# G1OJS/PyFT8

Measured on AMD Instinct MI355X. Metric: FT8 15-s frames decoded/sec, higher is better.
Workload: dtype f32

## Files before the change

pyft8_amd/csrc/ft8rx.hip:

```cpp
#include <hip/hip_runtime.h>
#include <math.h>
#include <stdarg.h>
#include <stdio.h>
#include <stdlib.h>
#include <string.h>
#include <algorithm>
#include <map>
#include <new>
#include <string>
#include <type_traits>
#include <utility>
#include <vector>
#include "../../include/ft8rx.h"
#include "ft8_dev.h"

#define WL_MULT(i) ((i) == WL_BP0 ? 5 : (i) == WL_OSDNAN ? 10 : 1)
#define NF0MAX (FT8RX_MAX_F0 > 1024 ? 2048 : 1024)

#include "kernels/common.hpp"
#include "kernels/spectrogram.hpp"
#include "kernels/sync_search.hpp"
#include "kernels/llr.hpp"
#include "kernels/ap_patterns.hpp"
#include "kernels/bp.hpp"
#include "kernels/cycle_spectrum.hpp"
#include "kernels/fine_sync.hpp"
#include "kernels/osd.hpp"
#include "kernels/ap_calls.hpp"
#include "kernels/recall.hpp"
#include "kernels/report.hpp"
#include "kernels/ddc.hpp"
#include "kernels/ddc_wide.hpp"
#include "kernels/ddc_rat.hpp"
#include "kernels/blanker.hpp"
#include "kernels/synth.hpp"
#include "kernels/subtract.hpp"
#include "kernels/probes.hpp"
#include "host_messages.hpp"
#include "batch_plan.hpp"
#include "ddc_ring.hpp"
#include "ddc_wide_ring.hpp"
#include "ddc_rat_ring.hpp"
#include "optins.hpp"
#include "ilp_launch.hpp"

#define EV_EAGER_BYTES ((size_t)1 << 20)
#define HIPCHK(h, x) do { hipError_t _e = (x); if (_e != hipSuccess) { set_err(h, "%s failed: %s (%s:%d)", #x, hipGetErrorString(_e), __FILE__, __LINE__); return -2; } } while (0)

static std::vector<uint32_t> osd_trial_table(int S, int D, int T) {
    std::vector<uint32_t> t;
    const uint32_t N = OSD_NONE;
// ... 184 lines not shown
    if (e != hipSuccess) { set_err(h, "hipHostMalloc(%zu bytes) failed: %s", n * sizeof(T), hipGetErrorString(e)); return -2; }
    h->pinned.push_back(q); *p = (T*)q; if (dev) *dev = (T*)d; return 0;
}

enum WsGroup { WS_STAGING, WS_STAGING2, WS_MASK, WS_RECALL, WS_REPORTS, WS_PACKED, WS_SUB, WS_SUBD, WS_ONES, WS_DDC, WS_BLANK };
struct FirstUse {
    ft8rx_handle* h; WsGroup g; size_t nd, nh; int rc = 0;
    std::vector<void**> members;
    FirstUse(ft8rx_handle* h_, WsGroup g_) : h(h_), g(g_), nd(h_->allocs.size()), nh(h_->pinned.size()) {}
    template <typename T> void dev(T** p, size_t n) { if (!rc && !(rc = dalloc(h, p, n))) members.push_back((void**)p); }
    template <typename T> void host(T** p, size_t n, T** d = nullptr) {
        if (rc || (rc = halloc(h, p, n, d))) return;
        members.push_back((void**)p); if (d) members.push_back((void**)d);
    }
    int done() {
        if (!rc) { h->ready |= 1u << g; return 0; }
        while (h->allocs.size() > nd) { hipFree(h->allocs.back()); h->allocs.pop_back(); }
        while (h->pinned.size() > nh) { hipHostFree(h->pinned.back()); h->pinned.pop_back(); }
        for (void** m : members) *m = nullptr;
        return -2;
    }
};
static bool ws_ready(const ft8rx_handle* h, WsGroup g) { return (h->ready >> g) & 1u; }
#define FIRST_HIP(F, x) do { if (!(F).rc) { hipError_t _e = (x); if (_e != hipSuccess) { set_err((F).h, "%s failed: %s (%s:%d)", #x, hipGetErrorString(_e), __FILE__, __LINE__); (F).rc = -2; } } } while (0)

static int need_staging(ft8rx_handle* h, bool second = false) {
    const WsGroup g = second ? WS_STAGING2 : WS_STAGING;
    if (ws_ready(h, g)) return 0;
    FirstUse F(h, g);
    F.dev(second ? &h->d_audio2 : &h->d_audio, (size_t)h->max_frames * FT8RX_NSAMP);
    return F.done();
}

static void host_twiddle(int n, int count, std::vector<cpx>& w) {
    w.resize(count);
    for (int t = 0; t < count; t++) {
        double ang = (2.0 * M_PI * (double)t) / (double)n;
        w[t] = make_float2((float)cos(ang), (float)(-sin(ang)));
    }
}
template <typename T> static int upload(ft8rx_handle* h, const T** dst, const std::vector<T>& v) {
    T* p; if (dalloc(h, &p, v.size())) return -2;
    if (hipMemcpy(p, v.data(), v.size() * sizeof(T), hipMemcpyHostToDevice) != hipSuccess) { set_err(h, "table upload failed"); return -2; }
    *dst = p; return 0;
}

struct Scratch {
    ft8rx_handle* h;
    ~Scratch() { for (auto& c : h->arena) c.used = 0; }
    void* raw(size_t bytes) {
        bytes = (bytes + 255) & ~(size_t)255;
        if (!bytes) bytes = 256;
        for (auto& c : h->arena) if (c.cap - c.used >= bytes) { void* q = (char*)c.p + c.used; c.used += bytes; return q; }
        size_t largest = 0;
        for (auto& c : h->arena) if (c.cap > largest) largest = c.cap;
        size_t cap = bytes > 2 * largest ? bytes : 2 * largest;
        if (cap < ((size_t)1 << 20)) cap = (size_t)1 << 20;
        for (size_t i = 0; i < h->arena.size();) {
            if (h->arena[i].used == 0) { hipFree(h->arena[i].p); h->arena.erase(h->arena.begin() + i); } else i++;
        }
        void* q = nullptr;
        if (hipMalloc(&q, cap) != hipSuccess) { if (cap == bytes || hipMalloc(&q, bytes) != hipSuccess) return nullptr; cap = bytes; }
        h->arena.push_back({q, cap, bytes});
        return q;
    }
    template <typename T> T* get(size_t n) { return (T*)raw(n * sizeof(T)); }
// ... 125 lines not shown
    for (int i = 0; i < WL_N; i++) rc |= dalloc(h, &h->d_work[i], B * S * WL_MULT(i));
    rc |= dalloc(h, &h->d_wcount, (size_t)batchplan::MAX_CHUNKS * WL_N);
    rc |= dalloc(h, &h->d_apc, batchplan::MAX_CHUNKS);
    rc |= dalloc(h, &h->d_apcount, (size_t)batchplan::MAX_CHUNKS * 2);
    rc |= dalloc(h, &h->d_ev, B * FT8RX_EVENT_CAP);
    rc |= dalloc(h, &h->d_evcount, B);
    ResultSlot* const sl = h->slots;
    sl[0].rec = h->d_rec; sl[0].ncand = h->d_ncand; sl[0].ev = h->d_ev; sl[0].evcount = h->d_evcount;
    rc |= dalloc(h, &sl[1].rec, B * S);
    rc |= dalloc(h, &sl[1].ncand, B);
    rc |= dalloc(h, &sl[1].ev, B * FT8RX_EVENT_CAP);
    rc |= dalloc(h, &sl[1].evcount, B);
    const bool ev_compact = B * FT8RX_EVENT_CAP * sizeof(ft8rx_event) > EV_EAGER_BYTES;
    for (int k = 0; k < 2 && ev_compact; k++) rc |= dalloc(h, &sl[k].d_evoffs, B + 1);
    for (int k = 0; k < 2 && !rc; k++) {
        rc = halloc(h, &sl[k].h_rec, B * cfg->max_cands);
        if (!rc) rc = halloc(h, &sl[k].h_cnt, B);
        if (!rc) rc = halloc(h, &sl[k].h_ev, B * FT8RX_EVENT_CAP);
        if (!rc) rc = halloc(h, &sl[k].h_evc, B);
        if (!rc && ev_compact) rc = halloc(h, &sl[k].h_evpacked, B * FT8RX_EVENT_CAP, &sl[k].d_evpacked);
    }
    if (rc) { g_create_err = h->err; ft8rx_destroy(h); return -2; }
    std::vector<float> win(3840);
    for (int i = 0; i < 3840; i++) win[i] = (float)(0.5 + 0.5 * cos(M_PI * (double)(2 * i + 1 - 3840) / 3839.0));
    std::vector<double> taper(100);
    { double step = (0.0 - M_PI) / 99.0; for (int i = 0; i < 100; i++) { double y = (i == 99) ? 0.0 : (double)i * step + M_PI; taper[i] = 0.5 * (1.0 + cos(y)); } }
    std::vector<cpx> w;
    rc |= upload(h, &h->T.win, win);
    rc |= upload(h, &h->T.taper, taper);
    host_twiddle(1920, 1920, w);   rc |= upload(h, &h->T.W1920, w);
    host_twiddle(3840, FT8RX_GRID_COLS, w);    rc |= upload(h, &h->T.WR3840, w);
    host_twiddle(3200, 3200, w);   rc |= upload(h, &h->T.W3200, w);
    host_twiddle(96000, 96000, w); rc |= upload(h, &h->T.W96000, w);
    host_twiddle(300, 300, w);     rc |= upload(h, &h->T.W300, w);
    host_twiddle(320, 320, w);     rc |= upload(h, &h->T.W320, w);
    host_twiddle(192000, FT8RX_SPEC_BINS, w); rc |= upload(h, &h->T.WR192k, w);
    host_twiddle(32, 32, w);       rc |= upload(h, &h->T.W32, w);
    {
        std::vector<float> k32(1800);
        std::vector<cpx> cs(156), g1000(1000);
        for (int m = -900; m < 900; m++) {
            const int r = ((m % 100) + 100) % 100;
            k32[m + 900] = (r == 0) ? (m == 0 ? 32.0f : 0.0f) : (float)(sin(M_PI * (double)r / 100.0) / sin(M_PI * (double)m / 3200.0));
        }
        for (int sidx = 1; sidx < 7; sidx++) for (int q = 0; q <= 25; q++) {
            const double a = 2.0 * M_PI * (double)((q * sidx) % 100) / 100.0;
            cpx v = make_float2((float)cos(a), (float)sin(a));
            if (q == 0) v = make_float2(1.0f, 0.0f);
            cs[(sidx - 1) * 26 + q] = v;
        }
        for (int k = -150; k < 850; k++) {
            const int r = ((k % 100) + 100) % 100, j = (k - r) / 100;
            const double a = M_PI * (31.0 * (double)r - 100.0 * (double)j) / 3200.0;
            g1000[k + 150] = make_float2((float)cos(a), (float)sin(a));
        }
        std::vector<cpx> tw100(100);
        for (int m = 0; m < 100; m++) { const double a = -2.0 * M_PI * (double)m / 100.0; tw100[m] = make_float2((float)cos(a), (float)sin(a)); }
        rc |= upload(h, &h->T.K32, k32); rc |= upload(h, &h->T.CS100, cs); rc |= upload(h, &h->T.G1000, g1000); rc |= upload(h, &h->T.TW100, tw100);
    }
    if (rc) { g_create_err = h->err; ft8rx_destroy(h); return -2; }
    bool ok = true;
    ok &= hipMemcpyToSymbol(HIP_SYMBOL(d_CHK_N), FT8_CHK_N, sizeof(FT8_CHK_N)) == hipSuccess;
    ok &= hipMemcpyToSymbol(HIP_SYMBOL(d_CHK_V), FT8_CHK_V, sizeof(FT8_CHK_V)) == hipSuccess;
    {
        static uint8_t ev[522], ec[522]; static uint16_t ve[174][3];
        auto slot = [](int e) { const int c = FT8_EDGE_C[e], j = e - FT8_CHK_E0[c]; return j < 6 ? 83 * j + c : 498 + (c - 59); };
        for (int e = 0; e < 522; e++) { ev[slot(e)] = FT8_EDGE_V[e]; ec[slot(e)] = FT8_EDGE_C[e]; }
        for (int v = 0; v < 174; v++) for (int k = 0; k < 3; k++) ve[v][k] = (uint16_t)slot(FT8_VAR_E[v][k]);
        ok &= hipMemcpyToSymbol(HIP_SYMBOL(d_EDGE_V), ev, sizeof(ev)) == hipSuccess;
// ... 151 lines not shown
    const ResultSlot& sl = h->slots[slot];
    const bool weak = h->weak;
    const ft8rx_config cw = weak ? weak_config(h) : h->cfg;
    const ft8rx_config& c = weak ? cw : h->cfg;
    const size_t F = (size_t)f0;
    const int sh = cand_shift(c); const size_t S = (size_t)1 << sh, FS = F * S;
    const int16_t* audio = d_audio + F * FT8RX_NSAMP;
    float* grid = h->d_grid + F * FT8RX_GRID_ROWS * FT8RX_GRID_COLS;
    float* bs = h->d_best_score + F * NF0MAX; int32_t* bh = h->d_best_h0 + F * NF0MAX;
    ft8rx_record* rec = sl.rec + FS; int32_t* ncand = sl.ncand + F;
    float* llr0 = h->d_llr0 + FS * 174; float* saved = h->d_saved + FS * 5 * 174;
    Att* att0 = h->d_att0 + FS * 5; Att* attG = h->d_attG + FS * 2; Att* attB = h->d_attB + FS * 5; Att* attO = h->d_attO + FS * 10;
    cpx* A = reinterpret_cast<cpx*>(grid); cpx* spec = A + (size_t)B * 96000;
    ft8rx_event* ev = sl.ev + F * FT8RX_EVENT_CAP; int32_t* evc = sl.evcount + F;
#define STAGE(name) do { if (prof) { hipEventRecord(h->pev[h->pnames.size()], s); h->pnames.push_back(name); } } while (0)
    int32_t* wc = h->d_wcount + WL_N * chunk;
    WorkList wl[WL_N];
    for (int i = 0; i < WL_N; i++) { wl[i].items = h->d_work[i] + FS * WL_MULT(i); wl[i].count = wc + i; }
    STAGE("spectrogram");
    ft8rx_ilp_spectrogram(B, s, audio, grid, h->T);
    STAGE("sync");
    launch_sync(grid, bs, bh, c, B, s, weak);
    STAGE("topk");
    k_topk<<<B, 1024, 0, s>>>(bs, bh, rec, ncand, c, evc, wc, h->use_mask ? h->d_colmask + F * NF0MAX : nullptr);
    STAGE("grid_llr");
    const unsigned mt = (unsigned)h->msg_types;
    launch_mt(k_grid_llr, k_grid_llr_ext, mt, XCD_GRID(B, c.max_cands), s, grid, rec, ncand, llr0, c, nullptr, nullptr, nullptr, att0, ev, evc, B);
    k_worklist_att<<<(B * S * 5 + 255) / 256, 256, 0, s>>>(rec, ncand, att0, B, sh, wl[WL_BP0]);
    STAGE("bp_grid");
    launch_mt(k_bp, k_bp_ext, mt, ladder_grid(h, B * c.max_cands * 5), s, 0, llr0, rec, ncand, nullptr, att0, nullptr, ev, evc, c, c.bp_nc0_a, c.bp_iters_a, wl[WL_BP0], 0, 5);
    STAGE("select0");
    k_select0<<<(B * S + 255) / 256, 256, 0, s>>>(rec, ncand, att0, B, sh, wl[WL_FINE]);
    STAGE("cycle_fft");
    k_cyc_a<<<dim3(40, B), 256, 0, s>>>(audio, A, h->T);
    k_cyc_bc<<<dim3(CYC_BC_GRID, B), 256, 0, s>>>(A, spec, h->T);
    STAGE("fine");
    launch_fine(h, c, weak, ladder_grid(h, B * c.max_cands), s, spec, rec, ncand, llr0, nullptr, nullptr, nullptr, nullptr, wl[WL_FINE],
                c.h0_lo < FT8RX_MIN_H0_FD || c.h0_hi > FT8RX_MAX_H0_FD + 1);
    k_worklist<<<(B * S + 255) / 256, 256, 0, s>>>(rec, ncand, B, sh, wl[WL_BP1]);
    STAGE("bp_fine");
    const auto bp_fine = [&](int n_variants, const WorkList& work, int v0) {
        launch_mt(k_bp, k_bp_ext, mt, B * c.max_cands * n_variants, s, 1, llr0, rec, ncand, attG, attB, saved, ev, evc, c, c.bp_nc0_b, c.bp_iters_b,
                  work, v0, n_variants);
    };
    if (h->ladder_mode == 0) {
        bp_fine(1, wl[WL_BP1], 0);
        k_select1<<<(B * S + 255) / 256, 256, 0, s>>>(0, rec, ncand, attG, attB, B, c, wl[WL_BP1B]);
        bp_fine(1, wl[WL_BP1B], 1);
        k_select1<<<(B * S + 255) / 256, 256, 0, s>>>(1, rec, ncand, attG, attB, B, c, wl[WL_BP1C]);
        bp_fine(3, wl[WL_BP1C], 2);
        STAGE("select1");
        k_select1<<<(B * S + 255) / 256, 256, 0, s>>>(2, rec, ncand, attG, attB, B, c, wl[WL_OSD]);
    } else {
        bp_fine(5, wl[WL_BP1], 0);
        STAGE("select1");
        k_select1<<<(B * S + 255) / 256, 256, 0, s>>>(3, rec, ncand, attG, attB, B, c, wl[WL_OSD]);
    }
    STAGE("osd");
    launch_osd(h, mt, ladder_grid(h, B * c.max_cands * 10), s, 0, llr0, saved, attB, rec, ncand, attO, ev, evc, h->d_trials, h->n_trials,
               osd_nflip(c.osd_single, c.osd_triple), c.osd_max_hd, sh, wl[WL_OSD], wl[WL_OSDNAN]);
    STAGE("select2");
    k_select2<<<(B * S + 255) / 256, 256, 0, s>>>(rec, ncand, attO, B, sh);
    if (h->ap.np) {
        STAGE("ap_calls");
        ApCalls* apc = h->d_apc + chunk;
        if (h->ap_chunk_version[chunk] != h->ap_version) {
            k_ap_stage<<<1, 64, 0, s>>>(apc, h->ap);
            h->ap_chunk_version[chunk] = h->ap_version;
// ... 1507 lines not shown
    return sync_scores(h, grid, B, f0_lo, f0_hi, score, h0_idx, true);
}

static std::vector<int32_t> pack_triples(int n, const int32_t* frame, const int32_t* f0_idx, const int32_t* h0_idx) {
    std::vector<int32_t> trip(3 * (size_t)n);
    for (int i = 0; i < n; i++) { trip[3 * i] = frame[i]; trip[3 * i + 1] = f0_idx[i]; trip[3 * i + 2] = h0_idx[i]; }
    return trip;
}

int ft8rx_llr_grid(ft8rx_handle* h, const float* grid, int B, int n, const int32_t* frame, const int32_t* f0_idx,
                   const int32_t* h0_idx, float* llr, float* sd, int32_t* snr) {
    if (!h || !grid || B < 1 || B > h->max_frames || n < 1) return -1;
    ENTER(h);
    HIPCHK(h, hipMemcpy(h->d_grid, grid, sizeof(float) * (size_t)B * FT8RX_GRID_ROWS * FT8RX_GRID_COLS, hipMemcpyHostToDevice));
    const std::vector<int32_t> trip = pack_triples(n, frame, f0_idx, h0_idx);
    Scratch S{h};
    int32_t* d_trip = S.put(trip.data(), trip.size()); NEED(d_trip);
    float* d_llr = S.get<float>((size_t)n * 174); NEED(d_llr);
    float* d_sd = S.get<float>(n); NEED(d_sd);
    int32_t* d_snr = S.get<int32_t>(n); NEED(d_snr);
    k_grid_llr<<<n, 64, 0, h->stream>>>(h->d_grid, nullptr, nullptr, d_llr, h->cfg, d_trip, d_sd, d_snr, nullptr, nullptr, nullptr, n);
    HIPCHK(h, hipStreamSynchronize(h->stream));
    HIPCHK(h, hipMemcpy(llr, d_llr, sizeof(float) * (size_t)n * 174, hipMemcpyDeviceToHost));
    HIPCHK(h, hipMemcpy(sd, d_sd, sizeof(float) * n, hipMemcpyDeviceToHost));
    HIPCHK(h, hipMemcpy(snr, d_snr, sizeof(int32_t) * n, hipMemcpyDeviceToHost));
    return 0;
}

int ft8rx_cycle_spectrum(ft8rx_handle* h, const int16_t* audio, int B, float* spec) {
    if (!h || !audio || !spec || B < 1 || B > h->max_frames) return -1;
    ENTER(h);
    if (need_staging(h)) return -2;
    HIPCHK(h, hipMemcpy(h->d_audio, audio, sizeof(int16_t) * (size_t)B * FT8RX_NSAMP, hipMemcpyHostToDevice));
    k_cyc_a<<<dim3(40, B), 256, 0, h->stream>>>(h->d_audio, h->d_A, h->T);
    k_cyc_bc<<<dim3(CYC_BC_GRID, B), 256, 0, h->stream>>>(h->d_A, h->d_spec, h->T);
    HIPCHK(h, hipStreamSynchronize(h->stream));
    HIPCHK(h, hipMemcpy(spec, h->d_spec, sizeof(cpx) * (size_t)B * FT8RX_SPEC_BINS, hipMemcpyDeviceToHost));
    return 0;
}

static int fine_probe(ft8rx_handle* h, const float* spec, int B, int n, const int32_t* frame, const int32_t* f0_idx, const int32_t* h0_idx,
                      int32_t* ret, int32_t* ttweak, int32_t* ftweak, int32_t* nsync, float* llr, float* sd, int32_t* snr, float* sgrid, bool weak) {
    if (!h || !spec || B < 1 || B > h->max_frames || n < 1) return -1;
    if (weak) for (int i = 0; i < n; i++)
        if (frame[i] < 0 || frame[i] >= B || f0_idx[i] < 4 || f0_idx[i] >= FT8RX_MAX_F0 || h0_idx[i] < FT8RX_MIN_H0 || h0_idx[i] >= FT8RX_MAX_H0) {
            set_err(h, "ft8rx_fine_weak: triple %d (frame %d, f0 %d, h0 %d) outside [0, %d) x [4, %d) x [%d, %d)", i,
                    frame[i], f0_idx[i], h0_idx[i], B, FT8RX_MAX_F0, FT8RX_MIN_H0, FT8RX_MAX_H0); return -1; }
    ENTER(h);
    HIPCHK(h, hipMemcpy(h->d_spec, spec, sizeof(cpx) * (size_t)B * FT8RX_SPEC_BINS, hipMemcpyHostToDevice));
    const std::vector<int32_t> trip = pack_triples(n, frame, f0_idx, h0_idx);
    Scratch S{h};
    int32_t* d_trip = S.put(trip.data(), trip.size()); NEED(d_trip);
    float* d_llr = S.get<float>((size_t)n * 174); NEED(d_llr);
    HIPCHK(h, hipMemset(d_llr, 0, sizeof(float) * (size_t)n * 174));
    float* d_sd = S.get<float>(n); NEED(d_sd);
    int32_t* d_out = S.get<int32_t>((size_t)n * 5); NEED(d_out);
    float* d_sg = sgrid ? S.get<float>((size_t)n * 632) : nullptr; if (sgrid) NEED(d_sg);
    launch_fine(h, weak ? weak_config(h) : h->cfg, weak, n, h->stream, h->d_spec, nullptr, nullptr, d_llr, d_trip, d_out, d_sd, d_sg,
                WorkList{nullptr, nullptr}, true);
    HIPCHK(h, hipStreamSynchronize(h->stream));
    std::vector<int32_t> o((size_t)n * 5);
    HIPCHK(h, hipMemcpy(o.data(), d_out, sizeof(int32_t) * o.size(), hipMemcpyDeviceToHost));
    for (int i = 0; i < n; i++) { ret[i] = o[5 * i]; ttweak[i] = o[5 * i + 1]; ftweak[i] = o[5 * i + 2]; nsync[i] = o[5 * i + 3]; snr[i] = o[5 * i + 4]; }
    HIPCHK(h, hipMemcpy(llr, d_llr, sizeof(float) * (size_t)n * 174, hipMemcpyDeviceToHost));
    HIPCHK(h, hipMemcpy(sd, d_sd, sizeof(float) * n, hipMemcpyDeviceToHost));
    if (sgrid) HIPCHK(h, hipMemcpy(sgrid, d_sg, sizeof(float) * (size_t)n * 632, hipMemcpyDeviceToHost));
    return 0;
}
// ... 313 lines not shown
    ENTER(h);
    HIPCHK(h, hipStreamSynchronize(h->stream));
    if (subtract_workspaces(h, 0)) return -2;
    if (h->sig_cap < max_sigs) {
        ft8rx_subsig* p = nullptr;
        if (dalloc(h, &p, (size_t)h->max_frames * max_sigs)) return -2;
        h->d_sigs = p; h->sig_cap = max_sigs;
    }
    int nmax = 0;
    for (int f = 0; f < B; f++) {
        if (counts[f] < 0 || counts[f] > max_sigs) { set_err(h, "ft8rx_subtract: counts[%d] = %d outside [0, %d]", f, counts[f], max_sigs); return -1; }
        if (counts[f] > nmax) nmax = counts[f];
    }
    HIPCHK(h, hipMemcpyAsync(h->d_sigs, sigs, sizeof(ft8rx_subsig) * (size_t)B * max_sigs, hipMemcpyHostToDevice, h->stream));
    HIPCHK(h, hipMemcpyAsync(h->d_sigcnt, counts, sizeof(int32_t) * B, hipMemcpyHostToDevice, h->stream));
    const size_t n = (size_t)B * FT8RX_NSAMP;
    k_sub_to_f32<<<(unsigned)((n + 255) / 256), 256, 0, h->stream>>>(d_audio, h->d_wf, n);
    if (subtract_workspaces(h, refine)) return -2;
    const SubTables T{h->d_pulse, h->d_pc};
    Tables Tones = h->T;
    if (refine == 3) Tones.taper = h->d_ones;
    for (int s = 0; s < nmax; s++) {
        const SubSel sel{h->d_sigs, h->d_sigcnt, max_sigs, s};
        if (refine == 2) {
            k_subd_mix<<<dim3(SUBD_NZ / 256, B), 256, 0, h->stream>>>(h->d_wf, sel, h->d_zdec, h->d_subctx);
            sub_refine(h, B, sel, T, true);
            k_subd_model<<<dim3((SUBD_N + 255) / 256, B), 256, 0, h->stream>>>(sel, T, h->d_subctx, h->d_model);
            k_subd_accum<<<B, 256, 0, h->stream>>>(h->d_zdec, h->d_model, sel, h->d_subctx, h->d_adec);
            k_subd_apply<<<dim3(SUB_GRIDX, B), 256, 0, h->stream>>>(h->d_wf, sel, T, h->d_adec);
            continue;
        }
        if (refine == 1) sub_refine(h, B, sel, T, false);
        if (refine == 3) {
            k_cyc_a_f32<<<dim3(40, B), 256, 0, h->stream>>>(h->d_wf, h->d_A, h->T);
            k_cyc_bc<<<dim3(CYC_BC_GRID, B), 256, 0, h->stream>>>(h->d_A, h->d_spec, h->T);
            k_refine3<<<B, FINE_NT, 0, h->stream>>>(h->d_spec, sel, Tones);
        }
        sub_apply_fullrate(h, B, sel, T);
    }
    k_sub_to_i16<<<(unsigned)((n + 255) / 256), 256, 0, h->stream>>>(h->d_wf, d_audio, n);
    HIPCHK(h, hipGetLastError());
    if (audio_f32_out) HIPCHK(h, hipMemcpyAsync(audio_f32_out, h->d_wf, sizeof(float) * n, hipMemcpyDeviceToHost, h->stream));
    if (refine) HIPCHK(h, hipMemcpyAsync(sigs, h->d_sigs, sizeof(ft8rx_subsig) * (size_t)B * max_sigs, hipMemcpyDeviceToHost, h->stream));
    HIPCHK(h, hipStreamSynchronize(h->stream));
    return 0;
}

int ft8rx_encode_tones(const uint64_t* msg_lo, const uint64_t* msg_hi, int n, uint8_t* tones) {
    if (!msg_lo || !msg_hi || !tones || n < 0) return -1;
    for (int i = 0; i < n; i++) hostmsg::encode_tones(msg_lo[i], msg_hi[i], tones + (size_t)i * 79);
    return 0;
}

void* ft8rx_alloc_host(ft8rx_handle* h, uint64_t bytes) {
    if (!h || bytes == 0) return nullptr;
    void* p = nullptr;
    if (hipSetDevice(h->device) != hipSuccess || hipHostMalloc(&p, (size_t)bytes, hipHostMallocDefault) != hipSuccess) {
        set_err(h, "ft8rx_alloc_host: hipHostMalloc(%llu) failed", (unsigned long long)bytes);
        return nullptr;
    }
    return p;
}

int ft8rx_free_host(ft8rx_handle* h, void* p) {
    if (!p) return -1;
    const hipError_t e = hipHostFree(p);
    if (e != hipSuccess) { if (h) set_err(h, "hipHostFree failed: %s", hipGetErrorString(e)); return -2; }
    return 0;
// ... 138 lines not shown
```

pyft8_amd/csrc/kernels/common.hpp:

```cpp
#ifndef FT8RX_COMMON_HPP
#define FT8RX_COMMON_HPP

struct Tables {
    const float* win;
    const cpx* W1920;
    const cpx* WR3840;
    const cpx* W3200;
    const cpx* W96000;
    const cpx* W300;
    const cpx* W320;
    const cpx* WR192k;
    const cpx* W32;
    const double* taper;
    const float* K32;
    const cpx* CS100;
    const cpx* TW100;
    const cpx* G1000;
};

__device__ __constant__ int d_COSTAS[7] = {3, 1, 4, 0, 6, 5, 2};
__device__ __constant__ uint8_t d_PAYSYM[58] = {7,8,9,10,11,12,13,14,15,16,17,18,19,20,21,22,23,24,25,26,27,28,29,30,31,32,33,34,35,
    43,44,45,46,47,48,49,50,51,52,53,54,55,56,57,58,59,60,61,62,63,64,65,66,67,68,69,70,71};
struct WorkList { int32_t* items; int32_t* count; };

constexpr __host__ __device__ int cand_shift(int max_cands) { return max_cands <= 256 ? 8 : max_cands <= 512 ? 9 : max_cands <= 1024 ? 10 : 11; }
constexpr __host__ __device__ int cand_shift(const ft8rx_config& c) { return cand_shift(c.max_cands); }
FT8_DEV bool cand_live(int c, int B, int sh, const int32_t* ncand) { return c < (B << sh) && (c & ((1 << sh) - 1)) < ncand[c >> sh]; }

FT8_DEV bool xcd_frame_map(int L, int per, int B, int& frame, int& idx) {
    const int x = L & 7, j = L >> 3;
    frame = 8 * (j / per) + x; idx = j % per;
    return frame < B;
}
#define XCD_GRID(B, per) ((((B) + 7) / 8) * 8 * (per))
enum { WL_BP0 = 0, WL_FINE = 1, WL_BP1 = 2, WL_BP1B = 3, WL_BP1C = 4, WL_OSD = 5, WL_OSDNAN = 6, WL_N = 7 };

#define W6 ((double)(-0.16666667163372040f))

#ifndef FT8RX_ILP_UNIT
__device__ __constant__ int8_t d_AP_CQ[29]   = {0,0,0,0,0, 0,0,0,0,0, 0,0,0,0,0, 0,0,0,0,0, 0,0,0,0,0, 0,1,0,0};
__device__ __constant__ int8_t d_AP_END[3][19] = {{0,1, 1,1,1,1,1, 0,0,1,1,1, 0,1,0,1,0, 0,1},
                                                  {0,1, 1,1,1,1,1, 0,1,0,0,1, 0,1,0,0,0, 0,1},
                                                  {0,1, 1,1,1,1,1, 0,1,0,0,1, 0,0,1,0,0, 0,1}};
__device__ uint8_t  d_CHK_N[83];
__device__ int16_t  d_CHK_V[83][7];
// ... 195 lines not shown
```

pyft8_amd/csrc/kernels/cycle_spectrum.hpp:

```cpp
#ifndef FT8RX_CYCLE_SPECTRUM_HPP
#define FT8RX_CYCLE_SPECTRUM_HPP

FT8_DEV uint32_t cyc_a_pair(const int16_t* __restrict__ a, int at, int inb) { return *reinterpret_cast<const uint32_t*>(a + at) & (uint32_t)inb; }
FT8_DEV float2 cyc_a_pair(const float* __restrict__ a, int at, int inb) {
    const float2 v = *reinterpret_cast<const float2*>(a + at);
    return make_float2(__uint_as_float(__float_as_uint(v.x) & (uint32_t)inb), __uint_as_float(__float_as_uint(v.y) & (uint32_t)inb));
}
FT8_DEV cpx cyc_a_point(uint32_t raw) { return make_float2((float)(int16_t)(raw & 0xFFFFu), (float)(int16_t)(raw >> 16)); }
FT8_DEV cpx cyc_a_point(float2 raw) { return raw; }
template <class In, class Raw> FT8_DEV void cyc_a_load(const In* __restrict__ a, int n2b, int tid, Raw (&raw)[10]) {
#pragma unroll
    for (int q = 0; q < 10; q++) {
        const int i = tid + 256 * q, ic = i < 2400 ? i : 0;
        const int c = ic & 7, n1 = ic >> 3;
        const int m = 320 * n1 + n2b + c;
        const int inb = (2 * m < FT8RX_NSAMP) ? -1 : 0;
        raw[q] = cyc_a_pair(a, (2 * m) & inb, inb);
    }
}
template <class Raw> FT8_DEV void cyc_a_frame(const Raw (&raw)[10], cpx* bufA, cpx* bufB, cpx* __restrict__ out, const Tables& T, int n2b, int tid) {
#pragma unroll
    for (int q = 0; q < 10; q++) {
        const int i = tid + 256 * q;
        if (i < 2400) bufA[(i & 7) * 300 + (i >> 3)] = cyc_a_point(raw[q]);
    }
    cpx w[10];
#pragma unroll
    for (int q = 0; q < 10; q++) { const int i = tid + 256 * q, ic = i < 2400 ? i : 0; w[q] = T.W96000[(n2b + (ic & 7)) * (ic >> 3)]; }
    __syncthreads();
    cpx* r = lds_fft<300, 5, 5, 4, 3>(bufA, bufB, T.W300, 8, tid, 256);
#pragma unroll
    for (int q = 0; q < 10; q++) {
        const int i = tid + 256 * q;
        if (i < 2400) { const int c = i & 7, k1 = i >> 3; out[k1 * 320 + n2b + c] = cmul(r[c * 300 + k1], w[q]); }
    }
}
__global__ __launch_bounds__(256) void k_cyc_a(const int16_t* __restrict__ audio, cpx* __restrict__ A, Tables T) {
    __shared__ cpx bufA[8 * 300];
    __shared__ cpx bufB[8 * 300];
    static_assert(320 / 8 == 8 * 5, "the tile map below assumes 40 column tiles = 8 XCDs x 5");
    const int tile = (blockIdx.x & 7) * 5 + (blockIdx.x >> 3);
    const int f = blockIdx.y, tid = threadIdx.x, n2b = 8 * tile;
    uint32_t raw[10];
    cyc_a_load(audio + (size_t)f * FT8RX_NSAMP, n2b, tid, raw);
    cyc_a_frame(raw, bufA, bufB, A + (size_t)f * 96000, T, n2b, tid);
}

#define CYC_BC_BLOCKS 39
#define CYC_BC_GRID 40
FT8_DEV int cyc_bc_row(int b, int r) {
    if (b == CYC_BC_BLOCKS - 1) return (r == 0) ? 0 : 150;
    const int k1a = 1 + 4 * b;
    return (r < 4) ? k1a + r : 300 - (k1a + (r - 4));
}
FT8_DEV void cyc_bc_load(const cpx* __restrict__ in, int b, int tid, cpx (&v)[10]) {
#pragma unroll
    for (int q = 0; q < 10; q++) {
        const int i = tid + 256 * q, r = i / 320, c = i - 320 * r;
        v[q] = in[(size_t)cyc_bc_row(b, r) * 320 + c];
    }
}
FT8_DEV void cyc_bc_frame(const cpx (&v)[10], cpx* bufA, cpx* bufB, cpx* __restrict__ out, const Tables& T, int b, int tid) {
#pragma unroll
    for (int q = 0; q < 10; q++) bufA[tid + 256 * q] = v[q];
    __syncthreads();
    cpx* z = lds_fft<320, 8, 8, 5>(bufA, bufB, T.W320, 8, tid, 256);
    const bool special = (b == CYC_BC_BLOCKS - 1);
    constexpr int NK2 = (FT8RX_SPEC_BINS + 299) / 300;
    static_assert(NK2 <= 320, "k2 range of the 320-point row transforms");
    for (int i = tid; i < 8 * NK2; i += 256) {
        const int half = i / (4 * NK2), j = i - half * (4 * NK2), rr = j & 3, k2 = j >> 2;
        const int r = 4 * half + rr;
        int pr, pk2;
        if (special) {
            if (r >= 2) continue;
            pr = r;
            pk2 = (r == 0) ? ((320 - k2) % 320) : 319 - k2;
        } else {
            pr = (r < 4) ? r + 4 : r - 4;
            pk2 = 319 - k2;
        }
        const int k = cyc_bc_row(b, r) + 300 * k2;
        if (k >= FT8RX_SPEC_BINS) continue;
        const cpx p = z[r * 320 + k2], q = z[pr * 320 + pk2];
        const float er = 0.5f * (p.x + q.x), ei = 0.5f * (p.y - q.y);
        const float orr = 0.5f * (p.y + q.y), oi = 0.5f * (q.x - p.x);
        const cpx w = T.WR192k[k];
        out[k] = make_float2(er + (w.x * orr - w.y * oi), ei + (w.x * oi + w.y * orr));
    }
}
__global__ __launch_bounds__(256) void k_cyc_bc(const cpx* __restrict__ A, cpx* __restrict__ spec, Tables T) {
    __shared__ cpx bufA[8 * 320];
    __shared__ cpx bufB[8 * 320];
    static_assert(CYC_BC_GRID == 8 * 5 && CYC_BC_BLOCKS <= CYC_BC_GRID, "tile map: 40 slots = 8 XCDs x 5");
    const int f = blockIdx.y, tid = threadIdx.x, b = (blockIdx.x & 7) * 5 + (blockIdx.x >> 3);
    if (b >= CYC_BC_BLOCKS) return;
    cpx v[10];
    cyc_bc_load(A + (size_t)f * 96000, b, tid, v);
    cyc_bc_frame(v, bufA, bufB, spec + (size_t)f * FT8RX_SPEC_BINS, T, b, tid);
}

#endif
```

pyft8_amd/csrc/kernels/subtract.hpp:

```cpp
#ifndef FT8RX_SUBTRACT_HPP
#define FT8RX_SUBTRACT_HPP

#define SUB_L (79 * 1920)
#define SUB_NCH 128
#define SUB_CH (SUB_L / SUB_NCH)

struct SubTables { const double* pulse; const double* pc; };

FT8_DEV void sub_signal(const ft8rx_subsig& S, const double* __restrict__ cum , const SubTables& T, int m, float* sr, float* si) {
    const int n = m + 1920;
    const double dphi_peak = 6.283185307179586 / 1920.0;
    int ih = n / 1920; if (ih > 78) ih = 78;
    const int il = ih - 2 > 0 ? ih - 2 : 0;
    double acc = cum[il] * T.pc[5759];
    for (int i = il; i <= ih; i++) {
        int j = n - 1920 * i; if (j > 5759) j = 5759;
        acc += (double)S.tones[i] * T.pc[j];
    }
    double phi = dphi_peak * acc + 6.283185307179586 * (S.fHz - 0.5) * (double)n / 12000.0;
    if (n < 3840) phi += dphi_peak * T.pulse[1920 + n] * (double)S.tones[0];
    if (n >= 79 * 1920) phi += dphi_peak * T.pulse[n - 79 * 1920] * (double)S.tones[78];
    const double rev = phi * (1.0 / 6.283185307179586);
    const float fr = (float)(rev - floor(rev));
    const float s = __builtin_amdgcn_sinf(fr), c = __builtin_amdgcn_cosf(fr);
// ... 324 lines not shown
        if (lane == 0) { pr[wave][k] = vr; pi_[wave][k] = vi; }
    }
    __syncthreads();
    if (tid < 20) {
        const double sc = ok ? (double)SUBD_D / 192000.0 : 0.0;
        Ar[tid] = (float)(((pr[0][tid] + pr[1][tid]) + (pr[2][tid] + pr[3][tid])) * sc);
        Ai[tid] = (float)(((pi_[0][tid] + pi_[1][tid]) + (pi_[2][tid] + pi_[3][tid])) * sc);
    }
    __syncthreads();
    for (int m = tid; m <= SUBD_N; m += 256) {
        const float rv = (float)(SUBD_D * m) * (1.0f / 192000.0f);
        float er, ei;
        sub_bins_synth(Ar, Ai, __builtin_amdgcn_cosf(rv), __builtin_amdgcn_sinf(rv), &er, &ei);
        adec[(size_t)frame * (SUBD_N + 1) + m] = make_float2(er, ei);
    }
}

__global__ __launch_bounds__(256) void k_subd_apply(float* __restrict__ wf, SubSel sel, SubTables T, const float2* __restrict__ adec) {
    __shared__ SubModel M;
    const int frame = blockIdx.y;
    int s0;
    if (!sub_begin(sel, frame, &M, &s0) || !sub_fits(s0)) return;
    float* x = wf + (size_t)frame * FT8RX_NSAMP + s0;
    const float2* a = adec + (size_t)frame * (SUBD_N + 1);
    sub_walk(M, T, [&](int m, float sr, float si) {
        int md = m >> 5; if (md > SUBD_N - 1) md = SUBD_N - 1;
        const float2 a0 = a[md], a1 = a[md + 1];
        float fq = (float)(m - SUBD_D * md) * (1.0f / 32.0f); if (fq > 1.0f) fq = 1.0f;
        const float er = a0.x + fq * (a1.x - a0.x), ei = a0.y + fq * (a1.y - a0.y);
        x[m] = x[m] - 2.0f * (er * sr - ei * si);
    });
}

__global__ __launch_bounds__(256) void k_cyc_a_f32(const float* __restrict__ audio, cpx* __restrict__ A, Tables T) {
    __shared__ cpx bufA[8 * 300];
    __shared__ cpx bufB[8 * 300];
    const int tile = (blockIdx.x & 7) * 5 + (blockIdx.x >> 3);
    const int f = blockIdx.y, tid = threadIdx.x, n2b = 8 * tile;
    float2 raw[10];
    cyc_a_load(audio + (size_t)f * FT8RX_NSAMP, n2b, tid, raw);
    cyc_a_frame(raw, bufA, bufB, A + (size_t)f * 96000, T, n2b, tid);
}

__global__ __launch_bounds__(FINE_NT) void k_refine3(const cpx* __restrict__ spec, SubSel sel, Tables T) {
    __shared__ cpx z[3200];
    __shared__ cpx slice[FINE_SLICE];
    __shared__ cpx w400[400];
    __shared__ cpx w32[32];
    __shared__ __attribute__((aligned(8))) double dsum[12 * 21 * 2];
    const int frame = blockIdx.x, tid = threadIdx.x;
    if (sel.s >= sel.counts[frame]) return;
    ft8rx_subsig& S = sel.sigs[(size_t)frame * sel.max_sigs + sel.s];
    const int fb0 = (int)(0.5 + S.fHz * 16.0);
    const int tb0 = (int)(0.5 + S.tsec * 200.0);
    if (fb0 - 182 < 0 || fb0 - 182 + FINE_SLICE > FT8RX_SPEC_BINS) return;
    const cpx* Sg = spec + (size_t)frame * FT8RX_SPEC_BINS + (fb0 - 182);
    for (int i = tid; i < FINE_SLICE; i += FINE_NT) slice[i] = Sg[i];
    for (int i = tid; i < 400; i += FINE_NT) w400[i] = T.W3200[8 * i];
    if (tid < 32) w32[tid] = T.W32[tid];
    __syncthreads();
    cpx wq[8];
    sym32_twiddles(w32, tid & 3, wq);
    FT_DECL
    fine_fft(slice, 182, z, w400, T, tid, 0, 3200 FT_PASS);
#pragma unroll 1
    for (int r = 0; r < (12 * 21 * 4 + FINE_NT - 1) / FINE_NT; r++) {
        const int task = tid + FINE_NT * r, qd = task >> 2, n2 = task & 3;
        const bool valid = qd < 12 * 21;
        const int ti = valid ? qd / 21 : 0, sy = valid ? qd - 21 * ti : 0;
        const int blk = sy / 7, a = sy - 7 * blk;
        float mag[8];
        fine_sym_quad<7>(z, tb0 - 6 + ti + 32 * (36 * blk + a), n2, wq, mag);
        if (valid && n2 == 0) { double on, off; fine_onoff(mag, a, on, off); dsum[(ti * 21 + sy) * 2] = on; dsum[(ti * 21 + sy) * 2 + 1] = off; }
    }
// ... 29 lines not shown
```

Baseline: 87230.

## Restructure cycle FFT kernels into 16-column register tiles with precomputed twiddle tables

```diff
diff --git a/pyft8_amd/csrc/cyc_index.hpp b/pyft8_amd/csrc/cyc_index.hpp
--- /dev/null
+++ b/pyft8_amd/csrc/cyc_index.hpp
@@ -0,0 +1,59 @@
+#pragma once
+#include <cstdint>
+
+#if defined(__HIPCC__)
+#define CYC_HD __host__ __device__ constexpr
+#else
+#define CYC_HD constexpr
+#endif
+
+namespace cycidx {
+
+constexpr int A_COLS = 16, A_TILES = 320 / A_COLS, A_BLOCK = 256, A_G1 = 12 * A_COLS, A_G2 = 25 * A_COLS, A_E = 12;
+constexpr int A_ROUNDS = (A_G2 + A_BLOCK - 1) / A_BLOCK;
+static_assert(A_TILES * A_COLS == 320 && A_G1 <= A_BLOCK && A_ROUNDS == 2, "20 tiles of 16 columns; one stage-1 group, two stage-2 groups per thread");
+CYC_HD int a_in_row(int g1, int jp, int j) { return g1 / A_COLS + 12 * jp + 60 * j; }
+struct APoint { int n2, k1; };
+CYC_HD APoint a_point(int tile, int g2, int e) {
+    return APoint{A_COLS * tile + g2 % A_COLS, g2 / A_COLS + 25 * (e % 4) + 100 * (e / 4)};
+}
+CYC_HD int a_pos(int tile, int g2, int e) { return (tile * A_E + e) * A_G2 + g2; }
+constexpr int A_TABLE = A_TILES * A_E * A_G2;
+
+constexpr int BC_BLOCKS = 20, BC_SLOTS = 16, BC_HALF = BC_SLOTS / 2, BC_BLOCK = 256, BC_B1 = 40 * BC_SLOTS, BC_G2 = 8 * BC_SLOTS;
+constexpr int BC_R1 = (BC_B1 + BC_BLOCK - 1) / BC_BLOCK;
+static_assert((BC_BLOCKS - 1) * BC_HALF == 152 && BC_R1 == 3 && BC_G2 <= BC_BLOCK, "19 blocks of 8 + 8 rows cover the rows 1 .. 299, one block the rows 0 and 150");
+CYC_HD int bc_nk2(int spec_bins) { return (spec_bins + 299) / 300; }
+CYC_HD int bc_row(int b, int r) {
+    if (b == BC_BLOCKS - 1) return (r == 0) ? 0 : 150;
+    const int k1a = 1 + BC_HALF * b;
+    return (r < BC_HALF) ? k1a + r : 300 - (k1a + (r - BC_HALF));
+}
+CYC_HD int bc_partner(int r) { return r < BC_HALF ? r + BC_HALF : r - BC_HALF; }
+struct BcSlot { int r, k2; };
+CYC_HD BcSlot bc_slot(int i, int nk2) {
+    const int half = i / (BC_HALF * nk2), j = i - half * (BC_HALF * nk2);
+    return BcSlot{BC_HALF * half + (j & (BC_HALF - 1)), j / BC_HALF};
+}
+CYC_HD int bc_bin(int b, int i, int nk2, int spec_bins) {
+    const BcSlot s = bc_slot(i, nk2);
+    if (b == BC_BLOCKS - 1 && s.r >= 2) return -1;
+    const int k = bc_row(b, s.r) + 300 * s.k2;
+    return k < spec_bins ? k : -1;
+}
+CYC_HD int bc_pos(int b, int i, int nk2) { return b * BC_SLOTS * nk2 + i; }
+CYC_HD int bc_table(int spec_bins) { return BC_BLOCKS * BC_SLOTS * bc_nk2(spec_bins); }
+CYC_HD int bc_sw(int i) { return i ^ ((i >> 3) & 7); }
+
+template <class C> inline void build_a_table(const C* W96000, C* out ) {
+    for (int t = 0; t < A_TILES; t++)
+        for (int g = 0; g < A_G2; g++)
+            for (int e = 0; e < A_E; e++) { const APoint p = a_point(t, g, e); out[a_pos(t, g, e)] = W96000[p.n2 * p.k1]; }
+}
+template <class C> inline void build_bc_table(const C* WR192k, int spec_bins, C unused, C* out ) {
+    const int nk2 = bc_nk2(spec_bins);
+    for (int b = 0; b < BC_BLOCKS; b++)
+        for (int i = 0; i < BC_SLOTS * nk2; i++) { const int k = bc_bin(b, i, nk2, spec_bins); out[bc_pos(b, i, nk2)] = k >= 0 ? WR192k[k] : unused; }
+}
+
+}
diff --git a/pyft8_amd/csrc/ft8rx.hip b/pyft8_amd/csrc/ft8rx.hip
--- a/pyft8_amd/csrc/ft8rx.hip
+++ b/pyft8_amd/csrc/ft8rx.hip
@@ -17,6 +17,7 @@
 #define WL_MULT(i) ((i) == WL_BP0 ? 5 : (i) == WL_OSDNAN ? 10 : 1)
 #define NF0MAX (FT8RX_MAX_F0 > 1024 ? 2048 : 1024)
 
+#include "cyc_index.hpp"
 #include "kernels/common.hpp"
 #include "kernels/spectrogram.hpp"
 #include "kernels/sync_search.hpp"
@@ -267,6 +268,13 @@
     return F.done();
 }
 
+static void launch_cyc_a(hipStream_t s, const int16_t* audio, cpx* A, const Tables& T, int B) { k_cyc_a<<<XCD_GRID(B, CYC_A_PER_FRAME), cycidx::A_BLOCK, 0, s>>>(audio, A, T, B); }
+static void launch_cyc_a(hipStream_t s, const float* audio, cpx* A, const Tables& T, int B) { k_cyc_a_f32<<<XCD_GRID(B, CYC_A_PER_FRAME), cycidx::A_BLOCK, 0, s>>>(audio, A, T, B); }
+template <class In> static void launch_cycle_fft(hipStream_t s, const In* audio, cpx* A, cpx* spec, const Tables& T, int B) {
+    launch_cyc_a(s, audio, A, T, B);
+    k_cyc_bc<<<XCD_GRID(B, CYC_BC_PER_FRAME), cycidx::BC_BLOCK, 0, s>>>(A, spec, T, B);
+}
+
 static void host_twiddle(int n, int count, std::vector<cpx>& w) {
     w.resize(count);
     for (int t = 0; t < count; t++) {
@@ -458,9 +466,17 @@
     host_twiddle(3840, FT8RX_GRID_COLS, w);    rc |= upload(h, &h->T.WR3840, w);
     host_twiddle(3200, 3200, w);   rc |= upload(h, &h->T.W3200, w);
     host_twiddle(96000, 96000, w); rc |= upload(h, &h->T.W96000, w);
+    {
+        std::vector<cpx> wo(cycidx::A_TABLE);
+        cycidx::build_a_table(w.data(), wo.data()); rc |= upload(h, &h->T.W96000o, wo);
+    }
     host_twiddle(300, 300, w);     rc |= upload(h, &h->T.W300, w);
     host_twiddle(320, 320, w);     rc |= upload(h, &h->T.W320, w);
     host_twiddle(192000, FT8RX_SPEC_BINS, w); rc |= upload(h, &h->T.WR192k, w);
+    {
+        std::vector<cpx> wo((size_t)cycidx::bc_table(FT8RX_SPEC_BINS));
+        cycidx::build_bc_table(w.data(), FT8RX_SPEC_BINS, make_float2(0.0f, 0.0f), wo.data()); rc |= upload(h, &h->T.WR192ko, wo);
+    }
     host_twiddle(32, 32, w);       rc |= upload(h, &h->T.W32, w);
     {
         std::vector<float> k32(1800);
@@ -678,8 +694,7 @@
     STAGE("select0");
     k_select0<<<(B * S + 255) / 256, 256, 0, s>>>(rec, ncand, att0, B, sh, wl[WL_FINE]);
     STAGE("cycle_fft");
-    k_cyc_a<<<dim3(40, B), 256, 0, s>>>(audio, A, h->T);
-    k_cyc_bc<<<dim3(CYC_BC_GRID, B), 256, 0, s>>>(A, spec, h->T);
+    launch_cycle_fft(s, audio, A, spec, h->T, B);
     STAGE("fine");
     launch_fine(h, c, weak, ladder_grid(h, B * c.max_cands), s, spec, rec, ncand, llr0, nullptr, nullptr, nullptr, nullptr, wl[WL_FINE],
                 c.h0_lo < FT8RX_MIN_H0_FD || c.h0_hi > FT8RX_MAX_H0_FD + 1);
@@ -2253,8 +2268,7 @@
     ENTER(h);
     if (need_staging(h)) return -2;
     HIPCHK(h, hipMemcpy(h->d_audio, audio, sizeof(int16_t) * (size_t)B * FT8RX_NSAMP, hipMemcpyHostToDevice));
-    k_cyc_a<<<dim3(40, B), 256, 0, h->stream>>>(h->d_audio, h->d_A, h->T);
-    k_cyc_bc<<<dim3(CYC_BC_GRID, B), 256, 0, h->stream>>>(h->d_A, h->d_spec, h->T);
+    launch_cycle_fft(h->stream, h->d_audio, h->d_A, h->d_spec, h->T, B);
     HIPCHK(h, hipStreamSynchronize(h->stream));
     HIPCHK(h, hipMemcpy(spec, h->d_spec, sizeof(cpx) * (size_t)B * FT8RX_SPEC_BINS, hipMemcpyDeviceToHost));
     return 0;
@@ -2634,8 +2648,7 @@
         }
         if (refine == 1) sub_refine(h, B, sel, T, false);
         if (refine == 3) {
-            k_cyc_a_f32<<<dim3(40, B), 256, 0, h->stream>>>(h->d_wf, h->d_A, h->T);
-            k_cyc_bc<<<dim3(CYC_BC_GRID, B), 256, 0, h->stream>>>(h->d_A, h->d_spec, h->T);
+            launch_cycle_fft(h->stream, h->d_wf, h->d_A, h->d_spec, h->T, B);
             k_refine3<<<B, FINE_NT, 0, h->stream>>>(h->d_spec, sel, Tones);
         }
         sub_apply_fullrate(h, B, sel, T);
diff --git a/pyft8_amd/csrc/kernels/common.hpp b/pyft8_amd/csrc/kernels/common.hpp
--- a/pyft8_amd/csrc/kernels/common.hpp
+++ b/pyft8_amd/csrc/kernels/common.hpp
@@ -11,6 +11,8 @@
     const cpx* W320;
     const cpx* WR192k;
     const cpx* W32;
+    const cpx* W96000o;
+    const cpx* WR192ko;
     const double* taper;
     const float* K32;
     const cpx* CS100;
diff --git a/pyft8_amd/csrc/kernels/cycle_spectrum.hpp b/pyft8_amd/csrc/kernels/cycle_spectrum.hpp
--- a/pyft8_amd/csrc/kernels/cycle_spectrum.hpp
+++ b/pyft8_amd/csrc/kernels/cycle_spectrum.hpp
@@ -1,6 +1,9 @@
 #ifndef FT8RX_CYCLE_SPECTRUM_HPP
 #define FT8RX_CYCLE_SPECTRUM_HPP
 
+#define CYC_A_PER_FRAME 20
+static_assert(CYC_A_PER_FRAME == cycidx::A_TILES && cycidx::A_COLS == 16 && cycidx::A_BLOCK == 256 && cycidx::A_G1 == 192 && cycidx::A_G2 == 400,
+              "cyc_a_tile below is written for 16-column tiles and 256 threads");
 FT8_DEV uint32_t cyc_a_pair(const int16_t* __restrict__ a, int at, int inb) { return *reinterpret_cast<const uint32_t*>(a + at) & (uint32_t)inb; }
 FT8_DEV float2 cyc_a_pair(const float* __restrict__ a, int at, int inb) {
     const float2 v = *reinterpret_cast<const float2*>(a + at);
@@ -8,96 +11,170 @@
 }
 FT8_DEV cpx cyc_a_point(uint32_t raw) { return make_float2((float)(int16_t)(raw & 0xFFFFu), (float)(int16_t)(raw >> 16)); }
 FT8_DEV cpx cyc_a_point(float2 raw) { return raw; }
-template <class In, class Raw> FT8_DEV void cyc_a_load(const In* __restrict__ a, int n2b, int tid, Raw (&raw)[10]) {
+template <class Raw, class In> FT8_DEV void cyc_a_tile(const In* __restrict__ a, cpx* __restrict__ out, cpx* z, const Tables& T, int tile, int tid) {
+    const cpx* __restrict__ W = T.W300;
+    const int n2b = cycidx::A_COLS * tile;
+    if (tid < cycidx::A_G1) {
+        const int c = tid & 15, p = tid >> 4;
+        Raw raw[5][5];
 #pragma unroll
-    for (int q = 0; q < 10; q++) {
-        const int i = tid + 256 * q, ic = i < 2400 ? i : 0;
-        const int c = ic & 7, n1 = ic >> 3;
-        const int m = 320 * n1 + n2b + c;
-        const int inb = (2 * m < FT8RX_NSAMP) ? -1 : 0;
-        raw[q] = cyc_a_pair(a, (2 * m) & inb, inb);
+        for (int jp = 0; jp < 5; jp++)
+#pragma unroll
+            for (int j = 0; j < 5; j++) {
+                const int m = 320 * cycidx::a_in_row(tid, jp, j) + n2b + c;
+                const int inb = (2 * m < FT8RX_NSAMP) ? -1 : 0;
+                raw[jp][j] = cyc_a_pair(a, (2 * m) & inb, inb);
+            }
+        cpx v[5][5];
+#pragma unroll
+        for (int jp = 0; jp < 5; jp++) {
+#pragma unroll
+            for (int j = 0; j < 5; j++) v[jp][j] = cyc_a_point(raw[jp][j]);
+            dft<5>(v[jp]);
+            const int p1 = p + 12 * jp;
+#pragma unroll
+            for (int j = 1; j < 5; j++) v[jp][j] = cmul(v[jp][j], W[j * p1]);
+        }
+#pragma unroll
+        for (int j = 0; j < 5; j++) {
+            cpx u[5];
+#pragma unroll
+            for (int jp = 0; jp < 5; jp++) u[jp] = v[jp][j];
+            dft<5>(u);
+#pragma unroll
+            for (int jp = 1; jp < 5; jp++) u[jp] = cmul(u[jp], W[jp * p * 5]);
+#pragma unroll
+            for (int jp = 0; jp < 5; jp++) z[(25 * p + 5 * jp + j) * 16 + c] = u[jp];
+        }
+    }
+    cpx w[cycidx::A_ROUNDS][cycidx::A_E];
+#pragma unroll
+    for (int r = 0; r < cycidx::A_ROUNDS; r++) {
+        const int g = tid + cycidx::A_BLOCK * r, gc = g < cycidx::A_G2 ? g : 0;
+#pragma unroll
+        for (int e = 0; e < cycidx::A_E; e++) w[r][e] = T.W96000o[cycidx::a_pos(tile, gc, e)];
+    }
+    __syncthreads();
+#pragma unroll
+    for (int r = 0; r < cycidx::A_ROUNDS; r++) {
+        const int g = tid + cycidx::A_BLOCK * r;
+        if (g >= cycidx::A_G2) break;
+        const int c = g & 15, q = g >> 4;
+        cpx v[3][4];
+#pragma unroll
+        for (int jp = 0; jp < 3; jp++)
+#pragma unroll
+            for (int j = 0; j < 4; j++) v[jp][j] = z[(q + 25 * (jp + 3 * j)) * 16 + c];
+#pragma unroll
+        for (int jp = 0; jp < 3; jp++) {
+            dft<4>(v[jp]);
+#pragma unroll
+            for (int j = 1; j < 4; j++) v[jp][j] = cmul(v[jp][j], W[j * jp * 25]);
+        }
+#pragma unroll
+        for (int j = 0; j < 4; j++) {
+            cpx u[3];
+#pragma unroll
+            for (int jp = 0; jp < 3; jp++) u[jp] = v[jp][j];
+            dft<3>(u);
+#pragma unroll
+            for (int jp = 0; jp < 3; jp++) out[(q + 25 * j + 100 * jp) * 320 + n2b + c] = cmul(u[jp], w[r][4 * jp + j]);
+        }
     }
 }
-template <class Raw> FT8_DEV void cyc_a_frame(const Raw (&raw)[10], cpx* bufA, cpx* bufB, cpx* __restrict__ out, const Tables& T, int n2b, int tid) {
-#pragma unroll
-    for (int q = 0; q < 10; q++) {
-        const int i = tid + 256 * q;
-        if (i < 2400) bufA[(i & 7) * 300 + (i >> 3)] = cyc_a_point(raw[q]);
-    }
-    cpx w[10];
-#pragma unroll
-    for (int q = 0; q < 10; q++) { const int i = tid + 256 * q, ic = i < 2400 ? i : 0; w[q] = T.W96000[(n2b + (ic & 7)) * (ic >> 3)]; }
-    __syncthreads();
-    cpx* r = lds_fft<300, 5, 5, 4, 3>(bufA, bufB, T.W300, 8, tid, 256);
-#pragma unroll
-    for (int q = 0; q < 10; q++) {
-        const int i = tid + 256 * q;
-        if (i < 2400) { const int c = i & 7, k1 = i >> 3; out[k1 * 320 + n2b + c] = cmul(r[c * 300 + k1], w[q]); }
-    }
-}
-__global__ __launch_bounds__(256) void k_cyc_a(const int16_t* __restrict__ audio, cpx* __restrict__ A, Tables T) {
-    __shared__ cpx bufA[8 * 300];
-    __shared__ cpx bufB[8 * 300];
-    static_assert(320 / 8 == 8 * 5, "the tile map below assumes 40 column tiles = 8 XCDs x 5");
-    const int tile = (blockIdx.x & 7) * 5 + (blockIdx.x >> 3);
-    const int f = blockIdx.y, tid = threadIdx.x, n2b = 8 * tile;
-    uint32_t raw[10];
-    cyc_a_load(audio + (size_t)f * FT8RX_NSAMP, n2b, tid, raw);
-    cyc_a_frame(raw, bufA, bufB, A + (size_t)f * 96000, T, n2b, tid);
+__global__ __launch_bounds__(256) void k_cyc_a(const int16_t* __restrict__ audio, cpx* __restrict__ A, Tables T, int B) {
+    __shared__ cpx z[16 * 300];
+    int f, tile;
+    if (!xcd_frame_map(blockIdx.x, CYC_A_PER_FRAME, B, f, tile)) return;
+    cyc_a_tile<uint32_t>(audio + (size_t)f * FT8RX_NSAMP, A + (size_t)f * 96000, z, T, tile, threadIdx.x);
 }
 
-#define CYC_BC_BLOCKS 39
-#define CYC_BC_GRID 40
-FT8_DEV int cyc_bc_row(int b, int r) {
-    if (b == CYC_BC_BLOCKS - 1) return (r == 0) ? 0 : 150;
-    const int k1a = 1 + 4 * b;
-    return (r < 4) ? k1a + r : 300 - (k1a + (r - 4));
-}
-FT8_DEV void cyc_bc_load(const cpx* __restrict__ in, int b, int tid, cpx (&v)[10]) {
+#define CYC_BC_PER_FRAME 20
+static_assert(CYC_BC_PER_FRAME == cycidx::BC_BLOCKS && cycidx::BC_SLOTS == 16 && cycidx::BC_BLOCK == 256 && cycidx::BC_R1 == 3 && cycidx::BC_G2 == 128,
+              "cyc_bc_block below is written for 8 + 8 rows and 256 threads");
+FT8_DEV void cyc_bc_block(const cpx* __restrict__ in, cpx* __restrict__ out, cpx* z, const Tables& T, int b, int tid) {
+    const cpx* __restrict__ W = T.W320;
+    {
+        cpx v[cycidx::BC_R1][8];
 #pragma unroll
-    for (int q = 0; q < 10; q++) {
-        const int i = tid + 256 * q, r = i / 320, c = i - 320 * r;
-        v[q] = in[(size_t)cyc_bc_row(b, r) * 320 + c];
+        for (int r = 0; r < 2; r++) {
+            const int b1 = tid + 256 * r, slot = b1 / 40, p = b1 - 40 * slot;
+            const cpx* __restrict__ x = in + (size_t)cycidx::bc_row(b, slot) * 320 + p;
+#pragma unroll
+            for (int j = 0; j < 8; j++) v[r][j] = x[40 * j];
+        }
+        if (tid < cycidx::BC_B1 - 512) {
+            const int b1 = tid + 512, slot = b1 / 40, p = b1 - 40 * slot;
+            const cpx* __restrict__ x = in + (size_t)cycidx::bc_row(b, slot) * 320 + p;
+#pragma unroll
+            for (int j = 0; j < 8; j++) v[2][j] = x[40 * j];
+        }
+#pragma unroll
+        for (int r = 0; r < cycidx::BC_R1; r++) {
+            const int b1 = tid + 256 * r, slot = b1 / 40, p = b1 - 40 * slot;
+            if (b1 < cycidx::BC_B1) {
+                dft<8>(v[r]);
+                z[slot * 320 + cycidx::bc_sw(8 * p)] = v[r][0];
+#pragma unroll
+                for (int j = 1; j < 8; j++) z[slot * 320 + cycidx::bc_sw(8 * p + j)] = cmul(v[r][j], W[j * p]);
+            }
+        }
     }
-}
-FT8_DEV void cyc_bc_frame(const cpx (&v)[10], cpx* bufA, cpx* bufB, cpx* __restrict__ out, const Tables& T, int b, int tid) {
+    __syncthreads();
+    if (tid < cycidx::BC_G2) {
+        const int slot = tid >> 3, q = tid & 7;
+        cpx* zr = z + slot * 320;
+        cpx v[5][8];
 #pragma unroll
-    for (int q = 0; q < 10; q++) bufA[tid + 256 * q] = v[q];
+        for (int p = 0; p < 5; p++)
+#pragma unroll
+            for (int j = 0; j < 8; j++) v[p][j] = zr[cycidx::bc_sw(q + 8 * (p + 5 * j))];
+#pragma unroll
+        for (int p = 0; p < 5; p++) {
+            dft<8>(v[p]);
+#pragma unroll
+            for (int j = 1; j < 8; j++) v[p][j] = cmul(v[p][j], W[j * p * 8]);
+        }
+#pragma unroll
+        for (int j = 0; j < 8; j++) {
+            cpx u[5];
+#pragma unroll
+            for (int p = 0; p < 5; p++) u[p] = v[p][j];
+            dft<5>(u);
+#pragma unroll
+            for (int p = 0; p < 5; p++) zr[cycidx::bc_sw(q + 8 * j + 64 * p)] = u[p];
+        }
+    }
     __syncthreads();
-    cpx* z = lds_fft<320, 8, 8, 5>(bufA, bufB, T.W320, 8, tid, 256);
-    const bool special = (b == CYC_BC_BLOCKS - 1);
-    constexpr int NK2 = (FT8RX_SPEC_BINS + 299) / 300;
+    const bool special = (b == cycidx::BC_BLOCKS - 1);
+    constexpr int NK2 = cycidx::bc_nk2(FT8RX_SPEC_BINS);
     static_assert(NK2 <= 320, "k2 range of the 320-point row transforms");
-    for (int i = tid; i < 8 * NK2; i += 256) {
-        const int half = i / (4 * NK2), j = i - half * (4 * NK2), rr = j & 3, k2 = j >> 2;
-        const int r = 4 * half + rr;
+    for (int i = tid; i < cycidx::BC_SLOTS * NK2; i += 256) {
+        const cycidx::BcSlot sl = cycidx::bc_slot(i, NK2);
+        const int r = sl.r, k2 = sl.k2;
         int pr, pk2;
         if (special) {
             if (r >= 2) continue;
             pr = r;
             pk2 = (r == 0) ? ((320 - k2) % 320) : 319 - k2;
         } else {
-            pr = (r < 4) ? r + 4 : r - 4;
+            pr = cycidx::bc_partner(r);
             pk2 = 319 - k2;
         }
-        const int k = cyc_bc_row(b, r) + 300 * k2;
+        const int k = cycidx::bc_row(b, r) + 300 * k2;
         if (k >= FT8RX_SPEC_BINS) continue;
-        const cpx p = z[r * 320 + k2], q = z[pr * 320 + pk2];
+        const cpx p = z[r * 320 + cycidx::bc_sw(k2)], q = z[pr * 320 + cycidx::bc_sw(pk2)];
         const float er = 0.5f * (p.x + q.x), ei = 0.5f * (p.y - q.y);
         const float orr = 0.5f * (p.y + q.y), oi = 0.5f * (q.x - p.x);
-        const cpx w = T.WR192k[k];
+        const cpx w = T.WR192ko[cycidx::bc_pos(b, i, NK2)];
         out[k] = make_float2(er + (w.x * orr - w.y * oi), ei + (w.x * oi + w.y * orr));
     }
 }
-__global__ __launch_bounds__(256) void k_cyc_bc(const cpx* __restrict__ A, cpx* __restrict__ spec, Tables T) {
-    __shared__ cpx bufA[8 * 320];
-    __shared__ cpx bufB[8 * 320];
-    static_assert(CYC_BC_GRID == 8 * 5 && CYC_BC_BLOCKS <= CYC_BC_GRID, "tile map: 40 slots = 8 XCDs x 5");
-    const int f = blockIdx.y, tid = threadIdx.x, b = (blockIdx.x & 7) * 5 + (blockIdx.x >> 3);
-    if (b >= CYC_BC_BLOCKS) return;
-    cpx v[10];
-    cyc_bc_load(A + (size_t)f * 96000, b, tid, v);
-    cyc_bc_frame(v, bufA, bufB, spec + (size_t)f * FT8RX_SPEC_BINS, T, b, tid);
+__global__ __launch_bounds__(256) void k_cyc_bc(const cpx* __restrict__ A, cpx* __restrict__ spec, Tables T, int B) {
+    __shared__ cpx z[16 * 320];
+    int f, b;
+    if (!xcd_frame_map(blockIdx.x, CYC_BC_PER_FRAME, B, f, b)) return;
+    cyc_bc_block(A + (size_t)f * 96000, spec + (size_t)f * FT8RX_SPEC_BINS, z, T, b, threadIdx.x);
 }
 
 #endif
diff --git a/pyft8_amd/csrc/kernels/subtract.hpp b/pyft8_amd/csrc/kernels/subtract.hpp
--- a/pyft8_amd/csrc/kernels/subtract.hpp
+++ b/pyft8_amd/csrc/kernels/subtract.hpp
@@ -380,14 +380,11 @@
     });
 }
 
-__global__ __launch_bounds__(256) void k_cyc_a_f32(const float* __restrict__ audio, cpx* __restrict__ A, Tables T) {
-    __shared__ cpx bufA[8 * 300];
-    __shared__ cpx bufB[8 * 300];
-    const int tile = (blockIdx.x & 7) * 5 + (blockIdx.x >> 3);
-    const int f = blockIdx.y, tid = threadIdx.x, n2b = 8 * tile;
-    float2 raw[10];
-    cyc_a_load(audio + (size_t)f * FT8RX_NSAMP, n2b, tid, raw);
-    cyc_a_frame(raw, bufA, bufB, A + (size_t)f * 96000, T, n2b, tid);
+__global__ __launch_bounds__(256) void k_cyc_a_f32(const float* __restrict__ audio, cpx* __restrict__ A, Tables T, int B) {
+    __shared__ cpx z[16 * 300];
+    int f, tile;
+    if (!xcd_frame_map(blockIdx.x, CYC_A_PER_FRAME, B, f, tile)) return;
+    cyc_a_tile<float2>(audio + (size_t)f * FT8RX_NSAMP, A + (size_t)f * 96000, z, T, tile, threadIdx.x);
 }
 
 __global__ __launch_bounds__(FINE_NT) void k_refine3(const cpx* __restrict__ spec, SubSel sel, Tables T) {
```

Measured after the change: 90030 (median of 6 runs). 1.03x the previous value.
